# ctu-mrs/mrs_uav_trajectory_generation

Measured on NVIDIA B200. Metric: optimized+sampled trajectories/sec (10-seg, N=10, fp64), higher is better.
Workload: dtype f64

## Files before the change

mrs_uav_trajectory_generation_b200/csrc/cuda_backend.cu:

```cuda
#include <cuda_runtime.h>

#include <cub/device/device_scan.cuh>
#include <cub/device/device_select.cuh>
#include <cub/iterator/counting_input_iterator.cuh>
#include <chrono>
#include <cstdlib>
#include <cstring>
#include <map>
#include <mutex>
#include <utility>
#include <vector>
#include <stdexcept>
#include <string>
#include <typeinfo>

#define TG_VERSION_STRING "tg_b200 0.1.0 (sm_100a, fp64, -fmad=false)"

#ifndef TG_JT_REFILL_REP
#define TG_JT_REFILL_REP 2
#endif
#include "tg_kernels.cuh"

namespace {

#define TG_CUDA_CHECK(expr)                                                                              \
  do {                                                                                                   \
    cudaError_t e__ = (expr);                                                                            \
    if (e__ != cudaSuccess)                                                                              \
      throw std::runtime_error(std::string(#expr) + ": " + cudaGetErrorString(e__));                     \
  } while (0)

template <class F, class = void>
struct MinBlocksOf {
  static constexpr int value = 1;
};
template <class F>
struct MinBlocksOf<F, decltype((void)F::kMinBlocks)> {
  static constexpr int value = F::kMinBlocks;
};
template <class F>
__global__ void __launch_bounds__(128, MinBlocksOf<F>::value) k_for_each(const F f, const size_t n) {
  const size_t i = (size_t)blockIdx.x * blockDim.x + threadIdx.x;
  if (i < n) f(i);
}

template <class F>
__global__ void __launch_bounds__(128) k_for_each_warp(const F f, const size_t n) {
  const size_t w = (size_t)blockIdx.x * 4 + (threadIdx.x >> 5);
  if (w < n) f(w, (int)(threadIdx.x & 31));
}

static_assert(TG_WARR_DEVICE_STRIDE == 32, "strided scratch kernels run one warp per block");
template <class F>
__global__ void __launch_bounds__(TG_WARR_DEVICE_STRIDE) k_for_each_scratch(const F f, const size_t n) {
  extern __shared__ double smem[];
  const size_t i = (size_t)blockIdx.x * blockDim.x + threadIdx.x;
  if (i < n) f(i, smem + threadIdx.x, (int)blockDim.x);
}

constexpr int kSolveWarps = 4;
template <class D>
__global__ void __launch_bounds__(kSolveWarps * 32) k_solve(const D desc, const size_t inst_begin, const size_t n_inst, const int ws_doubles, double* __restrict__ gws,
                                                            const int skip_oct_ws, const bool skip_thread) {
  extern __shared__ double smem[];
  const int warp = threadIdx.x >> 5, lane = threadIdx.x & 31;
  const size_t gw = (size_t)blockIdx.x * kSolveWarps + warp, nw = (size_t)gridDim.x * kSolveWarps;
  double* ws = gws ? gws + gw * (size_t)ws_doubles : smem + (size_t)warp * ws_doubles;
  for (size_t inst = inst_begin + gw; inst < n_inst; inst += nw) {
    tg::SolveInst I;
    if (!desc.instance(inst, I)) continue;
    if (skip_thread && tg::thread_eligible(I)) continue;
    if (skip_oct_ws > 0 && tg::octet_eligible(I) && tg::octet_ws_doubles(I.S, I.np) <= skip_oct_ws) continue;
    tg::solve_ws_bind(I, ws);
    tg::solve_warp(I, lane);
  }
}

template <class D>
__global__ void __launch_bounds__(32) k_solve_oct(const D desc, const size_t inst_begin, const size_t n_inst, const int oct_ws_doubles, const int u_cap,
                                                  double* __restrict__ uslab, const bool skip_thread) {
  extern __shared__ double smem[];
  const int lane = threadIdx.x & 31, oct = lane >> 3;
  const size_t gw = blockIdx.x, nw = gridDim.x;
  double* urows = uslab + ((size_t)blockIdx.x * 4 + oct) * (size_t)u_cap * tg::kOctURow;
  for (size_t base = inst_begin + gw * 4; base < n_inst; base += nw * 4) {
    tg::SolveInst I;
    const size_t inst = base + oct;
    bool ok = inst < n_inst && desc.instance(inst, I);
    if (ok && skip_thread && tg::thread_eligible(I)) ok = false;
    if (ok && !(tg::octet_eligible(I) && tg::octet_ws_doubles(I.S, I.np) <= oct_ws_doubles && I.np <= u_cap)) ok = false;
    if (!ok) {
      I.S = 0; I.np = 0; I.hbw = tg::kOctHbw; I.dp_out = nullptr; I.coef_out = nullptr; I.cost_out = nullptr;
    }
    const int nmax = __reduce_max_sync(0xffffffffu, I.np);
    if (nmax > 0) {
      tg::octet_ws_bind(I, smem + (size_t)oct * oct_ws_doubles, urows);
      tg::solve_octets(&I, lane, nmax);
    }
    __syncwarp();
  }
}

struct RefillLoad {
  int degree;
  double best;
};
template <int Q>
__device__ __noinline__ RefillLoad extrema_load_item(const double* __restrict__ c, const double T, double* __restrict__ p_lane) {
  typedef tg::QuantityJob<Q> Job;
  constexpr int M = Job::M;
  typename Job::Sink sink{c, T, TG_DBL_LOWEST};
  RefillLoad r{-1, TG_DBL_LOWEST};
  if (0.0 > T) return r;
  sink.consider(0.0);
  sink.consider(T);
  double ci[M + 1];
  if constexpr (Job::kPair) {
    constexpr int n_d = TG_N - Job::kDeriv, n_dd = n_d - 1, len = n_d + n_dd - 1;
#pragma unroll 1
    for (int i = 0; i < len; ++i) ci[i] = 0.0;
#pragma unroll 1
    for (int dim = 0; dim < 2; ++dim) {
      const double* cc = c + dim * TG_N;
      double dc[n_d], ddc[n_dd];
#pragma unroll 1
      for (int jx = 0; jx < n_d; ++jx) dc[jx] = cc[jx + Job::kDeriv] * tg::bcoef(Job::kDeriv, jx + Job::kDeriv);
#pragma unroll 1
      for (int jx = 0; jx < n_dd; ++jx) ddc[jx] = cc[jx + Job::kDeriv + 1] * tg::bcoef(Job::kDeriv + 1, jx + Job::kDeriv + 1);
#pragma unroll 1
      for (int i = 0; i < len; ++i) {
        double cv = 0.0;
        const int data_idx = i - n_dd + 1;
        const int lower = (0 > -data_idx) ? 0 : -data_idx, upper = (n_dd < n_d - data_idx) ? n_dd : n_d - data_idx;
#pragma unroll 1
        for (int kidx = lower; kidx < upper; ++kidx) cv = cv + ddc[n_dd - 1 - kidx] * dc[data_idx + kidx];
        ci[i] = ci[i] + cv;
      }
    }
  } else {
    const double* cc = c + Job::kD0 * TG_N;
#pragma unroll 1
    for (int jx = 0; jx <= M; ++jx) ci[jx] = cc[jx + Job::kDeriv + 1] * tg::bcoef(Job::kDeriv + 1, jx + Job::kDeriv + 1);
  }
  int last = -1;
#pragma unroll 1
  for (int i = 0; i <= M; i++)
    if (tg::dabs(ci[i]) >= TG_DBL_MIN) last = i;
  if (last >= 1) {
    int low = last;
#pragma unroll 1
    for (int i = M; i >= 0; i--)
      if (i <= last && ci[i] != 0.0) low = i;
    for (int z = 0; z < low; ++z) sink(0.0, 0.0);
    r.degree = last - low;
#pragma unroll 1
    for (int i = 0; i <= M; i++) {
      const int dst = last - i;
      if (dst >= 0 && dst <= r.degree) p_lane[dst * 32] = ci[i];
    }
  }
  r.best = sink.best;
  return r;
}

template <int Q>
__global__ void __launch_bounds__(32) k_extrema_refill(const double* __restrict__ coef, const double* __restrict__ times, double* __restrict__ maxima,
                                                       const int* __restrict__ work, const int* __restrict__ n_dev, const int n_max, int* __restrict__ counter,
                                                       unsigned long long* __restrict__ flop_counter) {
  extern __shared__ double smem[];
  typedef tg::QuantityJob<Q> Job;
  typedef typename Job::Sink Sink;
  constexpr int M = Job::M;
  const unsigned full = 0xffffffffu;
  const int lane = threadIdx.x & 31;
  const int n = n_dev ? min(n_max, *n_dev) : n_max;
  double* scratch = smem + lane;
  double svk[M + 1], tmp[M + 1];
  tg::JtMachine m;
  m.p = tg::WArr{scratch, 32};
  m.qp = tg::WArr{scratch + (size_t)(M + 1) * 32, 32};
  m.K = tg::WArr{scratch + (size_t)2 * (M + 1) * 32, 32};
  m.qk = tg::WArr{scratch + (size_t)3 * (M + 1) * 32, 32};
// ... 481 lines not shown
    const size_t grid = std::min(blocks_needed, (size_t)sm_count * thread_ctas_per_sm);
    const size_t need = grid * kThreadSolveCta * (size_t)rows_cap * tg::kThrRow;
    if (need > thread_slab_doubles) {
      if (thread_slab) {
        TG_CUDA_CHECK(cudaStreamSynchronize(stream));
        TG_CUDA_CHECK(cudaFree(thread_slab));
      }
      TG_CUDA_CHECK(cudaMalloc(&thread_slab, need * sizeof(double)));
      thread_slab_doubles = need;
    }
    const bool persist = l2_persist_bytes > 0 && n_inst > (size_t)4096;
    if (persist) {
      cudaStreamAttrValue av;
      std::memset(&av, 0, sizeof(av));
      const size_t bytes = std::min(need * sizeof(double), (size_t)l2_window_max);
      av.accessPolicyWindow.base_ptr = thread_slab;
      av.accessPolicyWindow.num_bytes = bytes;
      av.accessPolicyWindow.hitRatio = (float)std::min(1.0, (double)l2_persist_bytes / (double)bytes);
      av.accessPolicyWindow.hitProp = cudaAccessPropertyPersisting;
      av.accessPolicyWindow.missProp = cudaAccessPropertyStreaming;
      TG_CUDA_CHECK(cudaStreamSetAttribute(stream, cudaStreamAttributeAccessPolicyWindow, &av));
    }
    prof_begin();
    k_solve_thread<D><<<(unsigned)grid, kThreadSolveCta, 0, stream>>>(desc, inst_begin, inst_end, thread_slab);
    TG_CUDA_CHECK(cudaGetLastError());
    prof_end((std::string("thread:") + typeid(D).name()).c_str(), n_inst);
    if (persist) {
      cudaStreamAttrValue av;
      std::memset(&av, 0, sizeof(av));
      av.accessPolicyWindow.num_bytes = 0;
      TG_CUDA_CHECK(cudaStreamSetAttribute(stream, cudaStreamAttributeAccessPolicyWindow, &av));
    }
  }

  template <class D>
  void solve(size_t inst_begin, size_t inst_end, int ws_doubles, int oct_ws_doubles, int np_cap, bool mixed, const D& desc) {
    if (inst_end <= inst_begin) return;
    const size_t n_inst = inst_end - inst_begin;
    const int oct_warps = octet_warps_per_sm(oct_ws_doubles);
    if (oct_warps >= 1) {
      const size_t oct_smem = (size_t)4 * oct_ws_doubles * sizeof(double);
      prof_begin();
      allow_smem((const void*)k_solve_oct<D>, oct_smem);
      const size_t blocks_needed = (n_inst + 3) / 4;
      const size_t per_cta = (size_t)4 * std::max(np_cap, 1) * tg::kOctURow;
      size_t grid = std::min(blocks_needed, (size_t)sm_count * oct_warps);
      const size_t l2_ctas = std::max<size_t>((size_t)sm_count, ((size_t)96 << 20) / (per_cta * sizeof(double)));
      grid = std::min(grid, l2_ctas);
      double* us = slab(grid * per_cta);
      k_solve_oct<D><<<(unsigned)grid, 32, oct_smem, stream>>>(desc, inst_begin, inst_end, oct_ws_doubles, std::max(np_cap, 1), us, skip_thread_eligible);
      TG_CUDA_CHECK(cudaGetLastError());
      prof_end(typeid(D).name(), n_inst);
      if (!mixed) return;
    }
    const int skip = oct_warps >= 1 ? oct_ws_doubles : 0;
    const size_t ws_bytes = (size_t)ws_doubles * sizeof(double);
    const size_t smem = ws_bytes * kSolveWarps;
    const size_t blocks_needed = (n_inst + kSolveWarps - 1) / kSolveWarps;
    prof_begin();
    if (smem <= smem_optin) {
      allow_smem((const void*)k_solve<D>, smem);
      int per_sm = 0;
      TG_CUDA_CHECK(cudaOccupancyMaxActiveBlocksPerMultiprocessor(&per_sm, k_solve<D>, kSolveWarps * 32, smem));
      if (per_sm < 1) per_sm = 1;
      const size_t grid = std::min(blocks_needed, (size_t)sm_count * per_sm);
      k_solve<D><<<(unsigned)grid, kSolveWarps * 32, smem, stream>>>(desc, inst_begin, inst_end, ws_doubles, nullptr, skip, skip_thread_eligible);
    } else {
      const size_t grid = std::min(blocks_needed, (size_t)sm_count * 8);
      const size_t need = grid * kSolveWarps * (size_t)ws_doubles;
      if (need > gen_slab_doubles) {
        if (gen_slab) {
          TG_CUDA_CHECK(cudaStreamSynchronize(stream));
          TG_CUDA_CHECK(cudaFree(gen_slab));
        }
        TG_CUDA_CHECK(cudaMalloc(&gen_slab, need * sizeof(double)));
        gen_slab_doubles = need;
      }
      k_solve<D><<<(unsigned)grid, kSolveWarps * 32, 0, stream>>>(desc, inst_begin, inst_end, ws_doubles, gen_slab, skip, skip_thread_eligible);
    }
    TG_CUDA_CHECK(cudaGetLastError());
    prof_end(typeid(D).name(), n_inst);
  }

  void select_flagged(const uint8_t* flags, int* out, int* count, int n) {
    if (n <= 0) {
      TG_CUDA_CHECK(cudaMemsetAsync(count, 0, sizeof(int), stream));
      return;
    }
    cub::CountingInputIterator<int> idx(0);
    size_t bytes = 0;
    TG_CUDA_CHECK(cub::DeviceSelect::Flagged(nullptr, bytes, idx, flags, out, count, n, stream));
    if (bytes > scan_tmp_bytes) {
      if (scan_tmp) {
        TG_CUDA_CHECK(cudaStreamSynchronize(stream));
        TG_CUDA_CHECK(cudaFree(scan_tmp));
      }
      TG_CUDA_CHECK(cudaMalloc(&scan_tmp, bytes));
      scan_tmp_bytes = bytes;
    }
    TG_CUDA_CHECK(cub::DeviceSelect::Flagged(scan_tmp, bytes, idx, flags, out, count, n, stream));
  }
  void exclusive_scan(int* in, int* out, int n) {
    TG_CUDA_CHECK(cudaMemsetAsync(in + n, 0, sizeof(int), stream));
    size_t bytes = 0;
    TG_CUDA_CHECK(cub::DeviceScan::ExclusiveSum(nullptr, bytes, in, out, n + 1, stream));
    if (bytes > scan_tmp_bytes) {
      if (scan_tmp) {
        TG_CUDA_CHECK(cudaStreamSynchronize(stream));
        TG_CUDA_CHECK(cudaFree(scan_tmp));
      }
      TG_CUDA_CHECK(cudaMalloc(&scan_tmp, bytes));
      scan_tmp_bytes = bytes;
    }
    TG_CUDA_CHECK(cub::DeviceScan::ExclusiveSum(scan_tmp, bytes, in, out, n + 1, stream));
  }
};

#define TG_BACKEND CudaBackend
#include "tg_capi_impl.hpp"

extern "C" {

int tg_set_profiling(tg_ctx* ctx, int on) {
  if (!ctx) return TG_ERR_INVALID;
  ctx->be.profiling = on != 0;
  ctx->profiling = on != 0;
  ctx->be.prof.clear();
  return TG_OK;
}

int tg_get_profile(tg_ctx* ctx, int cap, char* names, int names_cap, double* ms, long long* launches, long long* items) {
  if (!ctx || !names || !ms || !launches || !items) return TG_ERR_INVALID;
  int n = 0;
  std::string all;
  for (const auto& kv : ctx->be.prof) {
    if (n >= cap) break;
    all += kv.first;
    all += "\n";
    ms[n] = kv.second.ms;
    launches[n] = kv.second.launches;
    items[n] = kv.second.items;
    ++n;
  }
  if ((int)all.size() + 1 > names_cap) return TG_ERR_INVALID;
  std::memcpy(names, all.c_str(), all.size() + 1);
  return n;
}

double tg_measure_fp64_peak(tg_ctx* ctx, int mode) {
  if (!ctx) return 0.0;
  try {
    return ctx->be.fp64_peak_tflops(mode);
  } catch (...) {
    return 0.0;
  }
}

}
```

mrs_uav_trajectory_generation_b200/csrc/tg_kernels.cuh:

```cuda
#ifndef TG_KERNELS_CUH_
#define TG_KERNELS_CUH_

#include "tg_common.cuh"
#include "tg_bound.cuh"
#include "tg_plis.cuh"
#include "tg_node.cuh"
#include "tg_poly.cuh"
#include "tg_segment.cuh"
#include "tg_solve.cuh"
#include "tg_solve_octet.cuh"
#include "tg_solve_thread.cuh"

#if defined(__CUDA_ARCH__)
#define TG_ATOMIC_MAX(p, v) atomicMax((p), (v))
#define TG_ATOMIC_ADD(p, v) atomicAdd((p), (v))
#define TG_ATOMIC_ADD_RET(p, v) atomicAdd((p), (v))
#elif defined(__CUDACC__)
#define TG_ATOMIC_MAX(p, v) ((void)0)
#define TG_ATOMIC_ADD(p, v) ((void)0)
#define TG_ATOMIC_ADD_RET(p, v) (0)
#else
static inline void tg_host_atomic_max(int* p, int v) {
  int cur = __atomic_load_n(p, __ATOMIC_RELAXED);
  while (cur < v && !__atomic_compare_exchange_n(p, &cur, v, true, __ATOMIC_RELAXED, __ATOMIC_RELAXED)) {
// ... 404 lines not shown
    I.rec_stride = 3;
    I.r = b.r;
    I.vmask = b.vmask + v0;
    I.vfree = b.vfree + v0 + p;
    I.vval = b.vval + (size_t)v0 * TG_HALF * TG_D;
    I.recs = b.recs + (size_t)s0 * 3 * TG_REC_SIZE;
    I.dp_out = nullptr;
    for (int k = t; k < total; k += 128) {
      const int n = k / per, it = k - n * per;
      I.variant = n;
      I.coef_out = (n == 0) ? b.coef + (size_t)s0 * TG_D * TG_N : nullptr;
      I.cost_out = b.costs + v0 + n;
      I.x_out = b.xs + (size_t)(v0 + n) * (size_t)b.xstride;
      f.run_instance(I, (size_t)(v0 + n) * (size_t)f.per_inst + it, it);
    }
  }
};
template <class D>
struct CostSumFn {
  D desc;
  int per_inst;
  const double* part;
  const int* inst_list = nullptr;
  TG_HD void operator()(size_t k) const {
    const size_t inst = inst_list ? (size_t)inst_list[k] : k;
    SolveInst I;
    if (!desc.instance(inst, I)) return;
    if (!I.cost_out) return;
    const double* pp = part + inst * (size_t)per_inst;
    double total = 0.0;
    for (int it = 0; it < I.S * TG_D; ++it) total += pp[it];
    *I.cost_out = 0.5 * total;
  }
};

TG_HD PlisVectors plis_vectors(const BatchPtrs& b, int p) {
  PlisVectors v;
  const int s0 = b.seg_off[p];
  v.x = b.x + s0;
  v.gf = b.g + s0;
  v.s = b.d + s0;
  v.xeval = b.xeval + s0;
  v.xo = b.hist_s + s0;
  v.go = b.hist_y + s0;
  v.ix = b.ix + s0;
  v.hstride = (size_t)b.totS;
  return v;
}
TG_HD void plis_enlist(const BatchPtrs& b, int p, int buf) {
  const int s0 = b.seg_off[p], S = b.seg_off[p + 1] - s0, v0 = s0 + p;
  int* cnt = b.stats + 9 + 3 * buf;
  const int jp = TG_ATOMIC_ADD_RET(&cnt[0], 1);
  b.act_prob[buf][jp] = p;
  const int jv = TG_ATOMIC_ADD_RET(&cnt[1], S + 1);
  for (int n = 0; n <= S; ++n) b.act_vtx[buf][jv + n] = v0 + n;
  const int js = TG_ATOMIC_ADD_RET(&cnt[2], S);
  for (int i = 0; i < S; ++i) b.act_seg[buf][js + i] = s0 + i;
}
struct PlisBeginFn {
  BatchPtrs b;
  int max_evals;
  TG_HD void operator()(size_t pi) const {
    const int p = (int)pi, s0 = b.seg_off[p], S = b.seg_off[p + 1] - s0;
    if (plis_begin(S, b.opt[p], plis_vectors(b, p), b.times + s0, max_evals)) plis_enlist(b, p, 0);
  }
};
struct PlisAdvanceFn {
  BatchPtrs b;
  int max_evals;
  double f_rel, x_rel;
  const int* prob_list;
  int next_buf;
  TG_HD void operator()(size_t k) const {
    const int p = prob_list ? prob_list[k] : (int)k, s0 = b.seg_off[p], S = b.seg_off[p + 1] - s0;
    PlisScalars& st = b.opt[p];
    if (st.done) return;
    plis_advance(S, st, plis_vectors(b, p), b.costs + vtx_off(b, p), max_evals, f_rel, x_rel, -1.0);
    if (!st.done) {
      TG_ATOMIC_ADD(&b.stats[7], 1);
      plis_enlist(b, p, next_buf);
    }
  }
};
struct PlisFinishFn {
  BatchPtrs b;
  TG_HD void operator()(size_t pi) const {
    const int p = (int)pi, s0 = b.seg_off[p], S = b.seg_off[p + 1] - s0;
    for (int i = 0; i < S; ++i) b.times[s0 + i] = b.xeval[s0 + i];
    ProbState& ps = b.ps[p];
    const PlisScalars& st = b.opt[p];
    ps.nlopt_code = st.code;
    ps.n_evals = st.n_evals;
    ps.n_grads = st.n_evals;
    ps.final_cost = st.f_last;
    if (st.n_evals == 0) ps.scale_done = 1;
    const int code = ps.nlopt_code;
    if (!((code >= 1 && code != 6) || code == -1)) ps.status = kFindNloptRejected;
  }
};

template <int Q>
struct ExtremaFn {
  BatchPtrs b;
  int* shift_count;
  static constexpr int kScratch = JtScratch<QuantityDegree<Q>::value>::kShared;
  TG_HD void operator()(size_t gs, double* scratch, int stride) const {
    const int p = b.prob_of_seg[gs];
    if (b.ps[p].scale_done) return;
    int shifts = 0;
    b.maxima[gs * 9 + Q] = segment_max_impl<Q>(b.coef + gs * TG_D * TG_N, b.times[gs], scratch, stride, &shifts);
    if (shift_count) TG_ATOMIC_ADD(shift_count, shifts);
  }
};
struct ExtremaWorkFn {
  const int* prob_of_seg;
  const ProbState* ps;
  const uint8_t* changed;
  uint8_t* flag;
  TG_HD void operator()(size_t gs) const { flag[gs] = (!ps[prob_of_seg[gs]].scale_done && changed[gs]) ? 1 : 0; }
};

struct ExtremaBoundFn {
  const double* coef;
  const double* times;
  double* maxima;
  uint8_t* is_bound;
  const int* work;
  const int* n_work;
  uint8_t* need;
  int list_stride;
  double L[9];
  double tol;
  TG_HD void operator()(size_t item) const {
    if (item >= (size_t)*n_work) return;
    const size_t gs = (size_t)work[item];
    for (int q = 0; q < 9; ++q) {
      const double thr = L[limit_index(q)] * (1.0 + tol) * (1.0 - 1e-12);
      const bool passes = (thr / L[limit_index(q)] <= 1.0 + tol) && certify_quantity_le(coef + gs * TG_D * TG_N, times[gs], q, thr);
      if (passes) {
        maxima[gs * 9 + q] = thr;
        is_bound[gs * 9 + q] = 1;
      } else {
        is_bound[gs * 9 + q] = 0;
        need[(size_t)q * list_stride + gs] = 1;
      }
    }
  }
};
TG_HD double prune_transform(int q, double ratio) {
  const int d = q % 3;
  return d == 0 ? ratio : (d == 1 ? dsqrt(ratio) : tgdm::dcbrt(ratio));
}
struct ExtremaPruneAFn {
  BatchPtrs b;
  double L[9];
  double* rq;
  uint8_t* qstar;
  uint8_t* need;
  int list_stride;
  TG_HD void operator()(size_t gs) const {
    const double* coef = b.coef + gs * TG_D * TG_N;
    const double T = b.times[gs];
    double bnd[9];
    segment_bounds(coef, T, bnd);
    double rmax = -1.0;
    int qs = -1;
// ... 559 lines not shown
```

mrs_uav_trajectory_generation_b200/csrc/tg_pipeline.hpp:

```cpp
#ifndef TG_PIPELINE_HPP_
#define TG_PIPELINE_HPP_

#include <algorithm>
#include <chrono>
#include <cstdio>
#include <cstdlib>
#include <cmath>
#include <cstring>
#include <functional>
#include <memory>
#include <string>
#include <vector>

#include "tg_kernels.cuh"
#include "tg_dfo.cuh"
#include "tg_dfo_generic.cuh"
#include "tg_generic.cuh"

namespace tg {

template <class BE>
class Arena {
 public:
  explicit Arena(BE& be, size_t chunk = (size_t)256 << 20) : be_(be), chunk_(chunk) {}
  ~Arena() {
    for (auto& c : chunks_) be_.dev_free(c.ptr);
  }
  void* alloc_bytes(size_t bytes) {
    bytes = (bytes + 255) & ~(size_t)255;
    if (bytes == 0) bytes = 256;
    while (cur_ < chunks_.size()) {
      Chunk& c = chunks_[cur_];
      if (c.used + bytes <= c.size) {
        void* p = (char*)c.ptr + c.used;
        c.used += bytes;
        return p;
      }
      ++cur_;
    }
    Chunk c;
    c.size = std::max(chunk_, bytes);
    c.ptr = be_.dev_alloc(c.size);
    c.used = bytes;
    chunks_.push_back(c);
    cur_ = chunks_.size() - 1;
    return c.ptr;
  }
  template <class T>
  T* alloc(size_t n) { return (T*)alloc_bytes(n * sizeof(T)); }
  void reset() {
    for (auto& c : chunks_) c.used = 0;
    cur_ = 0;
  }
  size_t bytes_reserved() const {
    size_t t = 0;
    for (auto& c : chunks_) t += c.size;
    return t;
  }

 private:
  struct Chunk { void* ptr; size_t size, used; };
  BE& be_;
  size_t chunk_;
  std::vector<Chunk> chunks_;
  size_t cur_ = 0;
};

struct Result {
  int status, success, nlopt_code, n_evals, rounds, safe, n_waypoints, n_samples, n_scale_passes, overflow;
  double max_dev, final_cost, baca_total;
  long long total_solves, total_root_calls, total_evals;
};

template <class T>
struct HostView {
  T* p = nullptr;
  size_t n = 0;
  T& operator[](size_t i) { return p[i]; }
  const T& operator[](size_t i) const { return p[i]; }
  T* data() { return p; }
  size_t size() const { return n; }
};

struct Group {
  int B = 0, totS = 0, totV = 0, totSlots = 0;
  std::vector<int> seg_off, smp_off;
  HostView<ProbState> ps;
  std::vector<int> orig;
  std::vector<int> h_np, h_hbw;
  int* d_seg_off = nullptr;
  double* d_wp = nullptr;
  uint8_t* d_stop = nullptr;
  double* d_init14 = nullptr;
  double* d_times = nullptr;
  double* d_coef = nullptr;
  double* d_xyzh = nullptr;
  int* d_smp_off = nullptr;
  uint8_t* d_seg_ok = nullptr;
  ProbState* d_ps = nullptr;
  BatchPtrs bp;
};

struct Counters {
  long long launches = 0, solves = 0, evals = 0, root_finds = 0, segment_setups = 0, samples = 0;
  double flops_solve = 0, flops_setup = 0, flops_sample = 0, flops_coef = 0;
  long long root_finds_executed = 0;
  long long mellinger_solves = 0, mellinger_launches = 0;
};

template <class BE>
class Pipeline {
 public:
  explicit Pipeline(BE& be) : be_(be), persist_(be), scratch_(be) {}

  BE& backend() { return be_; }
  Counters counters;
  bool prune_extrema = true;
  bool use_thread_solve = std::getenv("TG_NO_THREAD_SOLVE") == nullptr;
  size_t thread_min_inst = std::getenv("TG_THREAD_MIN_INST") ? (size_t)std::atoll(std::getenv("TG_THREAD_MIN_INST")) : (size_t)16384;
  bool thread_solve_for(size_t n_inst) const { return use_thread_solve && n_inst >= thread_min_inst; }
  size_t list_octet_below = std::getenv("TG_LIST_OCTET_BELOW") ? (size_t)std::atoll(std::getenv("TG_LIST_OCTET_BELOW")) : thread_min_inst;
  double scale_tolerance = 1e-3;
  size_t seg_budget = std::getenv("TG_SEG_BUDGET") ? (size_t)std::max(1LL, std::atoll(std::getenv("TG_SEG_BUDGET"))) : ((size_t)1 << 21);

  void find_group(Group& g, const Params& P, bool validate) {
    const int B = g.B, totS = g.totS, totV = g.totV;
    HostTrace tf0 = trace_mark();
    BatchPtrs& b = g.bp;
    std::memset(&b, 0, sizeof(b));
    b.B = B; b.totS = totS; b.totV = totV; b.r = P.derivative_to_optimize;
    b.seg_off = g.d_seg_off;
    b.wp = g.d_wp; b.stop = g.d_stop; b.init14 = g.d_init14;
    int* pov = scratch_.template alloc<int>(totV);
    int* pos = scratch_.template alloc<int>(totS);
    b.prob_of_vtx = pov; b.prob_of_seg = pos;
    b.vmask = scratch_.template alloc<uint8_t>(totV);
    b.vval = scratch_.template alloc<double>((size_t)totV * TG_HALF * TG_D);
    b.vfree = scratch_.template alloc<int>((size_t)totV + B);
    b.np = scratch_.template alloc<int>(B);
    b.hbw = scratch_.template alloc<int>(B);
    b.fmax = scratch_.template alloc<int>(B);
    b.stats = scratch_.template alloc<int>(16);
    b.times = g.d_times;
    b.baca = scratch_.template alloc<double>(totS);
    b.coef = g.d_coef;
    b.ps = g.d_ps;
    be_.dev_memset(b.stats, 0, 16 * sizeof(int));
    be_.for_each(B, VtxProblemFn{g.d_seg_off, pov, pos}); launches(1);
    be_.for_each(B, PrepareFn{b, 1}); launches(1);
    TimesFn tf{b, {}};
    for (int i = 0; i < 9; ++i) tf.L[i] = P.limits[i];
    be_.for_each(totS, tf); launches(1);
    be_.for_each(B, BacaTotalFn{b}); launches(1);
    int stats[16];
    be_.d2h(stats, b.stats, sizeof(stats));
    const int ws = stats[0], ows = stats[2];
    alloc_solution_buffers(b, (size_t)(P.run_time_alloc ? totV : B), stats);
    std::vector<int>& h_np = g.h_np;
    std::vector<int>& h_hbw = g.h_hbw;
    h_np.resize(B);
    h_hbw.resize(B);
    be_.d2h(h_np.data(), b.np, sizeof(int) * B);
    be_.d2h(h_hbw.data(), b.hbw, sizeof(int) * B);
    const std::vector<SolveBucket> buckets = make_buckets(B, g.seg_off.data(), h_np.data(), h_hbw.data(), ws, ows, stats[3]);
    trace_report(" find: prepare + buckets", -1, tf0);
    tf0 = trace_mark();
    if (P.run_time_alloc) {
      time_alloc_core(b, P, stats, &buckets);
      trace_report(" find: time allocation", -1, tf0);
      tf0 = trace_mark();
    } else {
      b.recs = scratch_.template alloc<double>((size_t)totS * TG_REC_SIZE);
    }
    be_.for_each(totS, SetupBaseFn{b, b.times});
    solve_with_outputs((size_t)B, stats, SolveProblemDesc{b, 0, nullptr, nullptr}, b, &buckets, false);
    launches(2);
    int* cap = scratch_.template alloc<int>((size_t)B + 1);
    g.d_smp_off = persist_.template alloc<int>((size_t)B + 1);
    be_.for_each(B, SampleCapFn{b, P.dt, cap}); launches(1);
    be_.exclusive_scan(cap, g.d_smp_off, B); launches(1);
    g.smp_off.resize(B + 1);
    be_.d2h(g.smp_off.data(), g.d_smp_off, sizeof(int) * (B + 1));
    g.totSlots = g.smp_off[B];
    const size_t slots = (size_t)std::max(g.totSlots, 1);
    int* seg_idx = scratch_.template alloc<int>(slots);
    int* smp_prob = scratch_.template alloc<int>(slots);
    double* t_in = scratch_.template alloc<double>(slots);
    g.d_xyzh = persist_.template alloc<double>(slots * 4);
    be_.for_each(B, SampleWalkFn{b, P.dt, g.d_smp_off, seg_idx, t_in});
    be_.for_each(B, SlotProblemFn{B, g.d_smp_off, smp_prob});
    be_.for_each((size_t)g.totSlots, SampleEvalFn{b, g.d_smp_off, smp_prob, seg_idx, t_in, g.d_xyzh, nullptr});
    be_.for_each(B, LengthCheckFn{b, P.dt, P.max_len_factor, P.min_len_factor});
    launches(4);
    if (P.override_heading_atan2) {
      be_.for_each(B, HeadingAtan2Fn{g.d_smp_off, g.d_ps, g.d_xyzh});
      launches(1);
    }
    if (validate) {
      be_.for_each(B, ValidateFn{g.bp, g.d_smp_off, g.d_xyzh, g.d_seg_ok, P.max_deviation, P.first_segment_checked, P.check_deviation});
      launches(1);
    }
    g.ps = HostView<ProbState>{static_cast<ProbState*>(be_.pinned_alloc(sizeof(ProbState) * (size_t)B)), (size_t)B};
    be_.d2h_pinned(g.ps.data(), g.d_ps, sizeof(ProbState) * B);
    trace_report(" find: solve .. state read", -1, tf0);
// ... 438 lines not shown
      const int ows = (hbw[p] == kOctHbw && np[p] >= kOctMinNp) ? octet_ws_doubles(S, np[p]) : 0;
      const int cls = be_.solve_class(ws, ows) * 4096 + (S + 3) / 4;
      if (out.empty() || cls != cls_prev) {
        if (out.size() >= 32) {
          out.assign(1, SolveBucket{0, B, 0, (size_t)seg_off[B] + B, ws_all, ows_all, np_all, 0, 0});
          mixed_single_ = true;
          return out;
        }
        out.push_back(SolveBucket{p, p, (size_t)seg_off[p] + p, 0, 0, 0, 0, 0, cls / 4096});
        cls_prev = cls;
      }
      SolveBucket& k = out.back();
      k.p1 = p + 1;
      k.v1 = (size_t)seg_off[p + 1] + p + 1;
      k.ws = std::max(k.ws, ws);
      k.ows = std::max(k.ows, ows);
      k.np_cap = std::max(k.np_cap, np[p]);
      k.s_cap = std::max(k.s_cap, S);
    }
    mixed_single_ = false;
    return out;
  }
  mutable bool mixed_single_ = false;
  template <class D>
  void solve_with_outputs(size_t n_inst, const int* stats, const D& desc, const BatchPtrs& b, const std::vector<SolveBucket>* buckets = nullptr,
                          bool per_vertex = false) {
    const bool use_thr = thread_solve_for(n_inst);
    const bool thread_all = use_thr && stats[8] == 0;
    if (use_thr) {
      be_.solve_thread(0, n_inst, kThrB * (std::max(b.smax, 1) + 1), desc);
      launches(1);
    }
    be_.skip_thread_eligible = use_thr;
    if (thread_all) {
    } else if (buckets && !buckets->empty()) {
      const bool mixed = mixed_single_;
      size_t a = 0;
      int n_launch = 0;
      while (a < buckets->size()) {
        SolveBucket m = (*buckets)[a];
        size_t e = a + 1;
        while (e < buckets->size() && (*buckets)[e].kernel_cls == m.kernel_cls) {
          const SolveBucket& k = (*buckets)[e];
          m.p1 = k.p1;
          m.v1 = k.v1;
          m.ws = std::max(m.ws, k.ws);
          m.ows = std::max(m.ows, k.ows);
          m.np_cap = std::max(m.np_cap, k.np_cap);
          ++e;
        }
        if (per_vertex) be_.solve(m.v0, m.v1, m.ws, m.ows, m.np_cap, mixed, desc);
        else be_.solve((size_t)m.p0, (size_t)m.p1, m.ws, m.ows, m.np_cap, mixed, desc);
        ++n_launch;
        a = e;
      }
      launches(n_launch - 1);
    } else {
      be_.solve(0, n_inst, stats[0], stats[2], stats[3], stats[6] > 0, desc);
    }
    const int per = 4 * b.smax;
    if (coef_cost_by_problem(n_inst, desc, b, buckets, per)) {
    } else if (buckets && buckets->size() > 1) {
      for (const SolveBucket& k : *buckets) {
        const size_t i0 = per_vertex ? k.v0 : (size_t)k.p0, i1 = per_vertex ? k.v1 : (size_t)k.p1;
        const int items = 4 * std::max(k.s_cap, 1);
        be_.for_each((i1 - i0) * (size_t)items, CoefCostFn<D>{desc, per, b.part, i0, items});
      }
      launches((int)buckets->size() - 1);
    } else {
      be_.for_each(n_inst * (size_t)per, CoefCostFn<D>{desc, per, b.part, 0, per});
    }
    be_.for_each(n_inst, CostSumFn<D>{desc, per, b.part, nullptr});
    launches(2);
  }

  template <class D>
  bool coef_cost_by_problem(size_t, const D&, const BatchPtrs&, const std::vector<SolveBucket>*, int) { return false; }
  bool coef_cost_by_problem(size_t, const SolveProblemDesc& desc, const BatchPtrs& b, const std::vector<SolveBucket>*, int per) {
    if (desc.mellinger != 1) return false;
    be_.for_each((size_t)b.B * 128, CoefCostGradFn{CoefCostFn<SolveProblemDesc>{desc, per, b.part, 0, per}, 0, nullptr});
    return true;
  }

  void time_alloc_core(BatchPtrs& b, const Params& P, const int* stats, const std::vector<SolveBucket>* buckets = nullptr) {
    const int B = b.B, totS = b.totS, totV = b.totV;
    const int mf = (P.max_evals > 0) ? std::min(std::max(P.max_evals, 1), kPlisMfMax) : kPlisMfMax;
    b.xeval = scratch_.template alloc<double>(totS);
    b.x = scratch_.template alloc<double>(totS);
    b.g = scratch_.template alloc<double>(totS);
    b.d = scratch_.template alloc<double>(totS);
    b.ix = scratch_.template alloc<int>(totS);
    b.hist_s = scratch_.template alloc<double>((size_t)mf * totS);
    b.hist_y = scratch_.template alloc<double>((size_t)mf * totS);
    b.opt = scratch_.template alloc<PlisScalars>(B);
    b.recs = scratch_.template alloc<double>((size_t)totS * 3 * TG_REC_SIZE);
    b.costs = scratch_.template alloc<double>(totV);
    b.maxima = scratch_.template alloc<double>((size_t)totS * 9);
    for (int k = 0; k < 2; ++k) {
      b.act_prob[k] = scratch_.template alloc<int>(B);
      b.act_vtx[k] = scratch_.template alloc<int>(totV);
      b.act_seg[k] = scratch_.template alloc<int>(totS);
    }
    be_.dev_memset(b.stats + 9, 0, 6 * sizeof(int));
    be_.for_each(B, PlisBeginFn{b, P.max_evals}); launches(1);
    const int eval_cap = (P.max_evals > 0 ? P.max_evals : 1000) + 64;
    int cnt[3] = {B, totV, totS};
    const bool lists_ok = thread_solve_for((size_t)totV) && stats[8] == 0;
    for (int e = 0; e < eval_cap; ++e) {
      const int buf = e & 1, nbuf = buf ^ 1;
      const bool sparse = lists_ok && e > 0 && (size_t)cnt[0] * 2 < (size_t)B;
      be_.dev_memset(b.stats + 7, 0, sizeof(int));
      be_.dev_memset(b.stats + 9 + 3 * nbuf, 0, 3 * sizeof(int));
      if (sparse) {
        const SolveProblemDesc desc{b, 1, nullptr, nullptr};
        const int per = 4 * b.smax;
        be_.for_each((size_t)cnt[2] * 3, SetupMellingerFn<0>{b, b.act_seg[buf]});
        be_.for_each((size_t)cnt[2] * 3 * TG_N, SetupMellingerFn<1>{b, b.act_seg[buf]});
        if ((size_t)cnt[1] >= list_octet_below) {
          be_.solve_thread(0, (size_t)cnt[1], kThrB * (std::max(b.smax, 1) + 1), SolveProblemListDesc{desc, b.act_vtx[buf]});
        } else {
          be_.skip_thread_eligible = false;
          be_.solve(0, (size_t)cnt[1], stats[0], stats[2], stats[3], stats[6] > 0, SolveProblemListDesc{desc, b.act_vtx[buf]});
        }
        be_.for_each((size_t)cnt[0] * 128, CoefCostGradFn{CoefCostFn<SolveProblemDesc>{desc, per, b.part, 0, per}, 0, b.act_prob[buf]});
        be_.for_each((size_t)cnt[1], CostSumFn<SolveProblemDesc>{desc, per, b.part, b.act_vtx[buf]});
        be_.for_each((size_t)cnt[0], PlisAdvanceFn{b, P.max_evals, P.f_rel, P.x_rel, b.act_prob[buf], nbuf});
        launches(6);
      } else {
        be_.for_each((size_t)totS * 3, SetupMellingerFn<0>{b, nullptr});
        be_.for_each((size_t)totS * 3 * TG_N, SetupMellingerFn<1>{b, nullptr});
        solve_with_outputs((size_t)totV, stats, SolveProblemDesc{b, 1, nullptr, nullptr}, b, buckets, true);
        be_.for_each(B, PlisAdvanceFn{b, P.max_evals, P.f_rel, P.x_rel, nullptr, nbuf});
        launches(4);
      }
      counters.mellinger_launches += 1;
      run_deferred();
      int back[8];
      be_.d2h(back, b.stats + 7, sizeof(back));
      if (back[0] == 0) break;
      cnt[0] = back[2 + 3 * nbuf];
      cnt[1] = back[3 + 3 * nbuf];
      cnt[2] = back[4 + 3 * nbuf];
    }
    be_.for_each(B, PlisFinishFn{b}); launches(1);
    scale_loop(b, P.limits);
  }

  bool time_alloc_batch(int B, const int* vtx_off, const uint8_t* vmask, const double* vval, double* times, const Params& P, double* coef,
                        int* nlopt_code, int* n_evals, int* n_scale_passes, double* final_cost) {
    scratch_.reset();
    std::vector<int> so(B + 1);
    for (int p = 0; p <= B; ++p) so[p] = vtx_off[p] - p;
    for (int p = 0; p < B; ++p)
      if (so[p + 1] - so[p] < 1) return false;
    Bare bb = bare_batch(B, so.data(), P.derivative_to_optimize);
    BatchPtrs& b = bb.b;
    b.vmask = scratch_.template alloc<uint8_t>(b.totV);
    b.vval = scratch_.template alloc<double>((size_t)b.totV * TG_HALF * TG_D);
    b.vfree = scratch_.template alloc<int>((size_t)b.totV + B);
    b.np = scratch_.template alloc<int>(B);
    b.hbw = scratch_.template alloc<int>(B);
    b.fmax = scratch_.template alloc<int>(B);
    b.times = scratch_.template alloc<double>(b.totS);
    b.coef = scratch_.template alloc<double>((size_t)b.totS * TG_D * TG_N);
    be_.h2d(b.vmask, vmask, b.totV);
    be_.h2d(b.vval, vval, sizeof(double) * (size_t)b.totV * TG_HALF * TG_D);
    be_.h2d(b.times, times, sizeof(double) * b.totS);
    be_.for_each(B, PrepareFn{b, 0}); launches(1);
    int stats[16];
    be_.d2h(stats, b.stats, sizeof(stats));
    alloc_solution_buffers(b, (size_t)b.totV, stats);
    time_alloc_core(b, P, stats);
    be_.for_each(b.totS, SetupBaseFn{b, b.times});
    solve_with_outputs((size_t)B, stats, SolveProblemDesc{b, 0, nullptr, nullptr}, b);
    launches(2);
    std::vector<ProbState> ps(B);
    be_.d2h(ps.data(), b.ps, sizeof(ProbState) * B);
    for (int p = 0; p < B; ++p) {
      if (nlopt_code) nlopt_code[p] = ps[p].nlopt_code;
      if (n_evals) n_evals[p] = ps[p].n_evals;
      if (n_scale_passes) n_scale_passes[p] = ps[p].n_scale_passes;
      if (final_cost) final_cost[p] = ps[p].final_cost;
      const int S = so[p + 1] - so[p];
      counters.evals += ps[p].n_evals;
      counters.solves += (long long)ps[p].n_evals * (S == 1 ? 1 : S + 1) + 1;
    }
    be_.d2h(times, b.times, sizeof(double) * b.totS);
    if (coef) be_.d2h(coef, b.coef, sizeof(double) * (size_t)b.totS * TG_D * TG_N);
    return true;
  }

  void preprocess_batch(int B, const int* wp_off, const double* wp, const uint8_t* stop, double min_dist, int straighten, double max_dev,
                        double max_hdg_dev, int* out_count, double* out_wp, uint8_t* out_stop) {
    scratch_.reset();
    const int totV = wp_off[B];
    int* d_off = scratch_.template alloc<int>((size_t)B + 1);
    double* d_wp = scratch_.template alloc<double>((size_t)std::max(totV, 1) * 4);
    uint8_t* d_stop = stop ? scratch_.template alloc<uint8_t>(std::max(totV, 1)) : nullptr;
    double* d_owp = scratch_.template alloc<double>((size_t)std::max(totV, 1) * 4);
    uint8_t* d_ostop = scratch_.template alloc<uint8_t>(std::max(totV, 1));
    int* d_cnt = scratch_.template alloc<int>(B);
    be_.h2d(d_off, wp_off, sizeof(int) * (B + 1));
    be_.h2d(d_wp, wp, sizeof(double) * 4 * (size_t)totV);
    if (stop) be_.h2d(d_stop, stop, totV);
    be_.for_each(B, PreprocessFn{d_off, d_wp, d_stop, min_dist, max_dev, max_hdg_dev, straighten, d_owp, d_ostop, d_cnt});
    launches(1);
    be_.d2h(out_count, d_cnt, sizeof(int) * B);
    if (out_wp) be_.d2h(out_wp, d_owp, sizeof(double) * 4 * (size_t)totV);
    if (out_stop) be_.d2h(out_stop, d_ostop, totV);
  }
  void fallback_batch(int B, const int* wp_off, const double* wp, const uint8_t* stop, const double* L9, double dt, double stopping_time, int* counts,
                      double* samples) {
    scratch_.reset();
    const int totV = wp_off[B];
    int* d_off = scratch_.template alloc<int>((size_t)B + 1);
    double* d_wp = scratch_.template alloc<double>((size_t)std::max(totV, 1) * 4);
    uint8_t* d_stop = stop ? scratch_.template alloc<uint8_t>(std::max(totV, 1)) : nullptr;
    double* d_vpos = scratch_.template alloc<double>((size_t)std::max(totV, 1) * 4);
    int* d_cnt = scratch_.template alloc<int>((size_t)B + 1);
    int* d_smp_off = scratch_.template alloc<int>((size_t)B + 1);
    be_.h2d(d_off, wp_off, sizeof(int) * (B + 1));
    be_.h2d(d_wp, wp, sizeof(double) * 4 * (size_t)totV);
    if (stop) be_.h2d(d_stop, stop, totV);
    FallbackFn f{d_off, d_wp, d_stop, {}, dt, stopping_time, d_vpos, d_cnt, nullptr, nullptr};
    for (int i = 0; i < 9; ++i) f.L[i] = L9[i];
    be_.for_each(B, f);
// ... 1407 lines not shown
```

Baseline: 407,500.

## Run small-tail Mellinger optimisation loop in one persistent per-problem kernel

When the number of active vertex instances falls below a threshold, the whole remaining optimisation loop (setup, octet solve, coefficient/cost, cost sum, line-search advance) runs inside a single kernel. Each block owns one problem and iterates all evaluations on the device with block-level syncs. This removes the per-evaluation multi-kernel launches and host round trips (d2h of stats) that dominate when few problems remain. The trade-off is lower parallelism per problem and heavy shared memory per block, plus optional host trace instrumentation.

```diff
diff --git a/mrs_uav_trajectory_generation_b200/csrc/cuda_backend.cu b/mrs_uav_trajectory_generation_b200/csrc/cuda_backend.cu
--- a/mrs_uav_trajectory_generation_b200/csrc/cuda_backend.cu
+++ b/mrs_uav_trajectory_generation_b200/csrc/cuda_backend.cu
@@ -98,6 +98,44 @@
       tg::solve_octets(&I, lane, nmax);
     }
     __syncwarp();
+  }
+}
+
+constexpr int kTailOctets = 16;
+__global__ void __launch_bounds__(kTailOctets * 8) k_mellinger_tail(const tg::MellingerTailFn f, const int* __restrict__ prob_list, const int n_prob,
+                                                                    const int max_evals, const int oct_ws_doubles, const int u_cap,
+                                                                    double* __restrict__ uslab) {
+  extern __shared__ double smem[];
+  const int t = threadIdx.x, lane = t & 31, oct = t >> 3;
+  double* ws = smem + (size_t)oct * oct_ws_doubles;
+  double* urows = uslab + ((size_t)blockIdx.x * kTailOctets + oct) * (size_t)u_cap * tg::kOctURow;
+  for (int k = blockIdx.x; k < n_prob; k += gridDim.x) {
+    const int p = prob_list ? prob_list[k] : k, S = f.segs(p);
+    for (int e = 0; e < max_evals && f.running(p); ++e) {
+      for (int i = t; i < 3 * S; i += blockDim.x) f.head(p, i);
+      __syncthreads();
+      for (int i = t; i < 3 * S * TG_N; i += blockDim.x) f.hrow(p, i);
+      __syncthreads();
+      for (int n0 = 0; n0 <= S; n0 += kTailOctets) {
+        tg::SolveInst I;
+        if (!f.instance(p, n0 + oct, I)) {
+          I.S = 0; I.np = 0; I.hbw = tg::kOctHbw; I.dp_out = nullptr; I.coef_out = nullptr; I.cost_out = nullptr;
+        }
+        const int nmax = __reduce_max_sync(0xffffffffu, I.np);
+        if (nmax > 0) {
+          tg::octet_ws_bind(I, ws, urows);
+          tg::solve_octets(&I, lane, nmax);
+        }
+        __syncwarp();
+      }
+      __syncthreads();
+      f.coef(p, t);
+      __syncthreads();
+      for (int n = t; n <= S; n += blockDim.x) f.cost_sum(p, n);
+      __syncthreads();
+      if (t == 0) f.advance(p);
+      __syncthreads();
+    }
   }
 }
 
@@ -745,6 +783,23 @@
     prof_end(typeid(D).name(), n_inst);
   }
 
+  bool mellinger_tail(const tg::MellingerTailFn& f, const int* prob_list, int n_prob, int max_evals, int oct_ws_doubles, int np_cap) {
+    const size_t smem = (size_t)kTailOctets * oct_ws_doubles * sizeof(double);
+    if (force_general_solve || oct_ws_doubles <= 0 || smem > smem_optin) return false;
+    if (n_prob <= 0) return true;
+    allow_smem((const void*)k_mellinger_tail, smem);
+    int per_sm = 0;
+    TG_CUDA_CHECK(cudaOccupancyMaxActiveBlocksPerMultiprocessor(&per_sm, k_mellinger_tail, kTailOctets * 8, smem));
+    const size_t grid = std::min((size_t)n_prob, (size_t)sm_count * std::max(per_sm, 1));
+    const int u_cap = std::max(np_cap, 1);
+    double* us = slab(grid * kTailOctets * (size_t)u_cap * tg::kOctURow);
+    prof_begin();
+    k_mellinger_tail<<<(unsigned)grid, kTailOctets * 8, smem, stream>>>(f, prob_list, n_prob, max_evals, oct_ws_doubles, u_cap, us);
+    TG_CUDA_CHECK(cudaGetLastError());
+    prof_end("k_mellinger_tail", (size_t)n_prob);
+    return true;
+  }
+
   void select_flagged(const uint8_t* flags, int* out, int* count, int n) {
     if (n <= 0) {
       TG_CUDA_CHECK(cudaMemsetAsync(count, 0, sizeof(int), stream));
diff --git a/mrs_uav_trajectory_generation_b200/csrc/tg_kernels.cuh b/mrs_uav_trajectory_generation_b200/csrc/tg_kernels.cuh
--- a/mrs_uav_trajectory_generation_b200/csrc/tg_kernels.cuh
+++ b/mrs_uav_trajectory_generation_b200/csrc/tg_kernels.cuh
@@ -510,6 +510,26 @@
     }
   }
 };
+struct MellingerTailFn {
+  BatchPtrs b;
+  int max_evals;
+  double f_rel, x_rel;
+  TG_HD SolveProblemDesc desc() const { return SolveProblemDesc{b, 1, nullptr, nullptr}; }
+  TG_HD int per() const { return 4 * b.smax; }
+  TG_HD int segs(int p) const { return b.seg_off[p + 1] - b.seg_off[p]; }
+  TG_HD bool running(int p) const { return !b.opt[p].done; }
+  TG_HD void head(int p, int k) const { SetupMellingerFn<0>{b, nullptr}((size_t)b.seg_off[p] * 3 + (size_t)k); }
+  TG_HD void hrow(int p, int k) const { SetupMellingerFn<1>{b, nullptr}((size_t)b.seg_off[p] * 3 * TG_N + (size_t)k); }
+  TG_HD bool instance(int p, int n, SolveInst& I) const { return n <= segs(p) && desc().instance((size_t)(vtx_off(b, p) + n), I); }
+  TG_HD void coef(int p, int t) const { CoefCostGradFn{CoefCostFn<SolveProblemDesc>{desc(), per(), b.part, 0, per()}, p, nullptr}((size_t)t); }
+  TG_HD void cost_sum(int p, int n) const { CostSumFn<SolveProblemDesc>{desc(), per(), b.part, nullptr}((size_t)(vtx_off(b, p) + n)); }
+  TG_HD void advance(int p) const {
+    PlisScalars& st = b.opt[p];
+    if (st.done) return;
+    plis_advance(segs(p), st, plis_vectors(b, p), b.costs + vtx_off(b, p), max_evals, f_rel, x_rel, -1.0);
+  }
+};
+
 struct PlisFinishFn {
   BatchPtrs b;
   TG_HD void operator()(size_t pi) const {
diff --git a/mrs_uav_trajectory_generation_b200/csrc/tg_pipeline.hpp b/mrs_uav_trajectory_generation_b200/csrc/tg_pipeline.hpp
--- a/mrs_uav_trajectory_generation_b200/csrc/tg_pipeline.hpp
+++ b/mrs_uav_trajectory_generation_b200/csrc/tg_pipeline.hpp
@@ -8,8 +8,11 @@
 #include <cmath>
 #include <cstring>
 #include <functional>
+#include <limits>
 #include <memory>
 #include <string>
+#include <type_traits>
+#include <utility>
 #include <vector>
 
 #include "tg_kernels.cuh"
@@ -18,6 +21,12 @@
 #include "tg_generic.cuh"
 
 namespace tg {
+
+template <class BE, class = void>
+struct HasMellingerTail : std::false_type {};
+template <class BE>
+struct HasMellingerTail<BE, std::void_t<decltype(std::declval<BE&>().mellinger_tail(std::declval<const MellingerTailFn&>(), (const int*)nullptr, 0, 0, 0, 0))>>
+    : std::true_type {};
 
 template <class BE>
 class Arena {
@@ -120,6 +129,7 @@
   size_t thread_min_inst = std::getenv("TG_THREAD_MIN_INST") ? (size_t)std::atoll(std::getenv("TG_THREAD_MIN_INST")) : (size_t)16384;
   bool thread_solve_for(size_t n_inst) const { return use_thread_solve && n_inst >= thread_min_inst; }
   size_t list_octet_below = std::getenv("TG_LIST_OCTET_BELOW") ? (size_t)std::atoll(std::getenv("TG_LIST_OCTET_BELOW")) : thread_min_inst;
+  size_t mellinger_tail_below = std::getenv("TG_MELLINGER_TAIL_BELOW") ? (size_t)std::atoll(std::getenv("TG_MELLINGER_TAIL_BELOW")) : list_octet_below;
   double scale_tolerance = 1e-3;
   size_t seg_budget = std::getenv("TG_SEG_BUDGET") ? (size_t)std::max(1LL, std::atoll(std::getenv("TG_SEG_BUDGET"))) : ((size_t)1 << 21);
 
@@ -724,6 +734,43 @@
     return true;
   }
 
+  bool mellinger_tail(const MellingerTailFn& f, const int* prob_list, int n_prob, int max_evals, int oct_ws_doubles, int np_cap) {
+    if constexpr (HasMellingerTail<BE>::value) {
+      return be_.mellinger_tail(f, prob_list, n_prob, max_evals, oct_ws_doubles, np_cap);
+    } else {
+      if (be_.solve_class(0, oct_ws_doubles) < 1) return false;
+      const int u_cap = std::max(np_cap, 1);
+      be_.for_each((size_t)std::max(n_prob, 0), [=](size_t k) {
+        const int p = prob_list ? prob_list[k] : (int)k, S = f.segs(p);
+        const double nan = std::numeric_limits<double>::quiet_NaN();
+        std::vector<double> ws((size_t)4 * oct_ws_doubles), us((size_t)4 * u_cap * kOctURow);
+        for (int e = 0; e < max_evals && f.running(p); ++e) {
+          for (int i = 0; i < 3 * S; ++i) f.head(p, i);
+          for (int i = 0; i < 3 * S * TG_N; ++i) f.hrow(p, i);
+          for (int n0 = 0; n0 <= S; n0 += 4) {
+            SolveInst I[4];
+            int nmax = 0;
+            std::fill(ws.begin(), ws.end(), nan);
+            std::fill(us.begin(), us.end(), nan);
+            for (int o = 0; o < 4; ++o) {
+              if (!f.instance(p, n0 + o, I[o])) {
+                I[o] = SolveInst{};
+                I[o].hbw = kOctHbw;
+              }
+              octet_ws_bind(I[o], ws.data() + (size_t)o * oct_ws_doubles, us.data() + (size_t)o * u_cap * kOctURow);
+              nmax = std::max(nmax, I[o].np);
+            }
+            if (nmax > 0) solve_octets(I, 0, nmax);
+          }
+          for (int t = 0; t < 128; ++t) f.coef(p, t);
+          for (int n = 0; n <= S; ++n) f.cost_sum(p, n);
+          f.advance(p);
+        }
+      });
+      return true;
+    }
+  }
+
   void time_alloc_core(BatchPtrs& b, const Params& P, const int* stats, const std::vector<SolveBucket>* buckets = nullptr) {
     const int B = b.B, totS = b.totS, totV = b.totV;
     const int mf = (P.max_evals > 0) ? std::min(std::max(P.max_evals, 1), kPlisMfMax) : kPlisMfMax;
@@ -748,10 +795,30 @@
     const int eval_cap = (P.max_evals > 0 ? P.max_evals : 1000) + 64;
     int cnt[3] = {B, totV, totS};
     const bool lists_ok = thread_solve_for((size_t)totV) && stats[8] == 0;
+    double tr_all = 0.0, tr_low = 0.0;
+    int tr_n = 0, tr_nlow = 0;
     for (int e = 0; e < eval_cap; ++e) {
+      const auto tr0 = std::chrono::steady_clock::now();
+      const bool tr_is_low = (size_t)cnt[1] < list_octet_below;
       const int buf = e & 1, nbuf = buf ^ 1;
       const bool sparse = lists_ok && e > 0 && (size_t)cnt[0] * 2 < (size_t)B;
       be_.dev_memset(b.stats + 7, 0, sizeof(int));
+      if (stats[6] == 0 && (size_t)cnt[1] < mellinger_tail_below &&
+          mellinger_tail(MellingerTailFn{b, P.max_evals, P.f_rel, P.x_rel}, e == 0 ? nullptr : b.act_prob[buf], e == 0 ? B : cnt[0],
+                         eval_cap - e, stats[2], stats[3])) {
+        launches(1);
+        counters.mellinger_launches += 1;
+        run_deferred();
+        if (be_.trace_host) {
+          be_.sync();
+          const double dt = std::chrono::duration<double>(std::chrono::steady_clock::now() - tr0).count();
+          tr_all += dt;
+          tr_low += dt;
+          ++tr_n;
+          ++tr_nlow;
+        }
+        break;
+      }
       be_.dev_memset(b.stats + 9 + 3 * nbuf, 0, 3 * sizeof(int));
       if (sparse) {
         const SolveProblemDesc desc{b, 1, nullptr, nullptr};
@@ -779,11 +846,20 @@
       run_deferred();
       int back[8];
       be_.d2h(back, b.stats + 7, sizeof(back));
+      if (be_.trace_host) {
+        const double dt = std::chrono::duration<double>(std::chrono::steady_clock::now() - tr0).count();
+        tr_all += dt;
+        ++tr_n;
+        if (tr_is_low) { tr_low += dt; ++tr_nlow; }
+      }
       if (back[0] == 0) break;
       cnt[0] = back[2 + 3 * nbuf];
       cnt[1] = back[3 + 3 * nbuf];
       cnt[2] = back[4 + 3 * nbuf];
     }
+    if (be_.trace_host)
+      std::fprintf(stderr, "[tg]   evaluations: %d in %7.2f ms; below %zu instances: %d in %7.2f ms (B %d, totV %d)\n", tr_n, 1e3 * tr_all,
+                   list_octet_below, tr_nlow, 1e3 * tr_low, B, totV);
     be_.for_each(B, PlisFinishFn{b}); launches(1);
     scale_loop(b, P.limits);
   }
```

Measured after the change: 413,000 (median of 6 runs). 1.01x the previous value.
